# EBI-Metagenomics/deciphon

Measured on AMD Instinct MI355X. Metric: GCUPS (Viterbi DP cell updates/sec), higher is better.
Workload: dtype f32

## Files before the change

deciphon_amd/csrc/engine.cpp:

```cpp
#include "../../include/deciphon_hip.h"
#include "dcp_db.h"
#include "dcp_errors.h"
#include "dcp_types.h"
#include "host_logic.h"
#include "viterbi_kernels.h"

#include <algorithm>
#include <atomic>
#include <deque>
#include <math.h>
#include <stdio.h>
#include <stdlib.h>
#include <string.h>
#include <string>
#include <thread>
#include <vector>

namespace
{

template <class T> struct DevBuf
{
  T *p = nullptr;
  size_t cap = 0;
// ... 121 lines not shown
  size_t trellis_off = 0;
  bool has_trellis = false;
  bool trellis_on_host = false;
  uint32_t const *steps = nullptr;
  int32_t nsteps = 0;
  std::vector<uint32_t> owned;
};

}

struct dcp_hip
{
  int device = 0;
  hipStream_t stream = nullptr;
  hipStream_t qstream[DCP_NUM_CLASSES] = {nullptr};
  hipEvent_t fork_ev = nullptr, join_ev[DCP_NUM_CLASSES] = {nullptr};
  hipStream_t pstream[DCP_NUM_PACK_SHAPES] = {nullptr};
  hipEvent_t pjoin_ev[DCP_NUM_PACK_SHAPES] = {nullptr};
  hipStream_t nstream[DCP_NUM_CLASSES] = {nullptr};
  hipEvent_t njoin_ev[DCP_NUM_CLASSES] = {nullptr};
  std::string err;

  std::vector<HostProfile> profiles;
  size_t committed = 0;
  DevBuf<float> d_pool;
  size_t pool_used = 0;
  int load_chunks = 0;
  DevBuf<DcpProfileDev> d_profiles;

  std::vector<int64_t> seq_off, row_off;
  DevBuf<unsigned char> d_nt;
  DevBuf<int64_t> d_seq_off, d_row_off;
  DevBuf<DcpCodeRow> d_rows;

  bool mode_set = false;
  bool multi_hits = true, hmmer3_compat = false;
  DevBuf<float> d_xt;
  int xt_rows = 0;
  std::vector<float> xt_override;

  struct Bank
  {
    DevBuf<DcpProblem> d_problems;
    DevBuf<DcpPack> d_packs;
    DevBuf<int2> d_pack_groups;
    DevBuf<float> d_out;
    DevBuf<uint32_t> d_hits;
    DevBuf<float> d_ring;
    PinBuf<uint32_t> h_hits;
    hipEvent_t done_ev = nullptr;
    int n = -1;
    PinBuf<DcpProblem> h_problems;
    PinBuf<DcpPack> h_packs;
    PinBuf<int2> h_groups;
    hipEvent_t up_ev = nullptr;
    bool up_pending = false;
  };
  Bank bank[3];
  int cur = 0;
  int outstanding[2] = {-1, -1};
  hipStream_t upload_stream = nullptr;
  struct StreamSet
  {
    hipStream_t stream = nullptr, qstream[DCP_NUM_CLASSES] = {nullptr};
    hipEvent_t fork_ev = nullptr, join_ev[DCP_NUM_CLASSES] = {nullptr};
  } path_set;
// ... 318 lines not shown
  {
    HIP_TRY(x, B.h_problems.reserve((size_t)nu), DCP_ENOMEM);
    memcpy(B.h_problems.p, st.problems.data(), (size_t)nu * sizeof(DcpProblem));
    HIP_TRY(x, hipMemcpyAsync(B.d_problems.p, B.h_problems.p, (size_t)nu * sizeof(DcpProblem), hipMemcpyHostToDevice, origin),
            DCP_EFUNCUSE);
  }
  if (!st.packs.empty())
  {
    HIP_TRY(x, B.h_packs.reserve(st.packs.size()), DCP_ENOMEM);
    memcpy(B.h_packs.p, st.packs.data(), st.packs.size() * sizeof(DcpPack));
    HIP_TRY(x, hipMemcpyAsync(B.d_packs.p, B.h_packs.p, st.packs.size() * sizeof(DcpPack), hipMemcpyHostToDevice, origin),
            DCP_EFUNCUSE);
  }
  if (!st.pack_groups.empty())
  {
    HIP_TRY(x, B.h_groups.reserve(st.pack_groups.size()), DCP_ENOMEM);
    memcpy(B.h_groups.p, st.pack_groups.data(), st.pack_groups.size() * sizeof(int2));
    HIP_TRY(x, hipMemcpyAsync(B.d_pack_groups.p, B.h_groups.p, st.pack_groups.size() * sizeof(int2), hipMemcpyHostToDevice,
                              origin),
            DCP_EFUNCUSE);
  }
  HIP_TRY(x, hipEventRecord(B.up_ev, origin), DCP_EFUNCUSE);
  B.up_pending = true;
  return 0;
}

DcpLaunch launch_args(dcp_hip *x, Staged const &st, int c)
{
  DcpLaunch a;
  a.pool = x->d_pool.p;
  a.profiles = x->d_profiles.p;
  a.problems = BK(x).d_problems.p + st.c_begin[c];
  a.code_rows = x->d_rows.p;
  a.xt_table = x->d_xt.p;
  a.out = BK(x).d_out.p;
  a.arena = x->d_trellis.p;
  a.nprob = st.c_begin[c + 1] - st.c_begin[c];
  a.stream = x->stream;
  a.ring = BK(x).d_ring.p;
  return a;
}

int launch_all(dcp_hip *x, Staged const &st, bool path)
{
  int classes = 0;
  for (int c = 0; c < DCP_NUM_CLASSES; ++c) classes += st.c_begin[c + 1] > st.c_begin[c];
  bool const fork = classes > 1;
  if (fork) HIP_TRY(x, hipEventRecord(x->fork_ev, x->stream), DCP_EFUNCUSE);
  std::vector<hipEvent_t> joins;
  for (int c = 0; c < DCP_NUM_CLASSES; ++c)
  {
    DcpLaunch a = launch_args(x, st, c);
    if (a.nprob <= 0) continue;
    if (path && c == DCP_STRIP_CLASS) continue;
    if (fork)
    {
      a.stream = x->qstream[c];
      HIP_TRY(x, hipStreamWaitEvent(a.stream, x->fork_ev, 0), DCP_EFUNCUSE);
    }
    HIP_TRY(x, path ? dcp_launch_path(c, a) : dcp_launch_cost(c, a), DCP_EFUNCUSE);
    if (fork)
    {
      HIP_TRY(x, hipEventRecord(x->join_ev[c], a.stream), DCP_EFUNCUSE);
      joins.push_back(x->join_ev[c]);
    }
  }
  for (hipEvent_t ev : joins) HIP_TRY(x, hipStreamWaitEvent(x->stream, ev, 0), DCP_EFUNCUSE);
  return 0;
}

int launch_cost_all(dcp_hip *x, Staged const &st, hipStream_t origin = nullptr, int reps = 1)
{
  if (!origin) origin = x->stream;
  int const single_wave = st.c_begin[4] - st.c_begin[0];
  int mixed = 0;
  for (int c = 0; c < 4; ++c) mixed += st.c_begin[c + 1] > st.c_begin[c];
  bool const fused = mixed >= 2 && single_wave <= 16384;
  int kernels = fused ? 1 : 0;
  for (int c = fused ? 4 : 0; c < DCP_NUM_CLASSES; ++c) kernels += st.c_begin[c + 1] > st.c_begin[c];
  for (int s = 0; s < DCP_NUM_PACK_SHAPES; ++s) kernels += st.pk_begin[s + 1] > st.pk_begin[s];
  char const *narrow_env = getenv("DECIPHON_HIP_NARROW");
  bool const narrow = !(narrow_env && narrow_env[0] == '0');
  for (int c = 4; narrow && c < DCP_NUM_CLASSES; ++c) kernels += st.c_wide[c] > st.c_begin[c];
  bool const fork = kernels > 1 || origin != x->stream;
  if (fork) HIP_TRY(x, hipEventRecord(x->fork_ev, origin), DCP_EFUNCUSE);
  std::vector<hipEvent_t> joins;
  for (int c = DCP_NUM_CLASSES - 1; c >= (fused ? 4 : 0); --c)
  {
    DcpLaunch b = launch_args(x, st, c);
    if (b.nprob <= 0) continue;
    if (fork)
    {
      b.stream = x->qstream[c];
      HIP_TRY(x, hipStreamWaitEvent(b.stream, x->fork_ev, 0), DCP_EFUNCUSE);
    }
    int const nn = narrow ? st.c_wide[c] - st.c_begin[c] : 0;
    if (nn > 0)
    {
      DcpLaunch n = b;
      n.nprob = nn;
      if (fork)
      {
        n.stream = x->nstream[c];
        HIP_TRY(x, hipStreamWaitEvent(n.stream, x->fork_ev, 0), DCP_EFUNCUSE);
      }
      for (int r = 0; r < reps; ++r) HIP_TRY(x, dcp_launch_cost_narrow(c, n), DCP_EFUNCUSE);
      if (fork)
      {
        HIP_TRY(x, hipEventRecord(x->njoin_ev[c], n.stream), DCP_EFUNCUSE);
        joins.push_back(x->njoin_ev[c]);
      }
      b.problems += nn;
      b.nprob -= nn;
    }
    if (b.nprob > 0)
      for (int r = 0; r < reps; ++r) HIP_TRY(x, dcp_launch_cost(c, b), DCP_EFUNCUSE);
    if (fork)
// ... 450 lines not shown
    dev[i].W = hp.W;
    dev[i].rows_off = hp.pool_off;
    dev[i].trans_off = dev[i].rows_off + (int64_t)DCP_TABLE_SIZE * (hp.Kp + DCP_ROW_HDR);
    dev[i].pad0 = dev[i].pad1 = 0;
  }
  HIP_TRY(x, x->d_profiles.reserve(dev.size()), DCP_ENOMEM);
  HIP_TRY(x, hipMemcpyAsync(x->d_profiles.p, dev.data(), dev.size() * sizeof(DcpProfileDev), hipMemcpyHostToDevice,
                            x->stream),
          DCP_EFUNCUSE);
  HIP_TRY(x, hipStreamSynchronize(x->stream), DCP_EFUNCUSE);
  x->committed = x->profiles.size();
  return 0;
}

void dcp_hip_clear_profiles(struct dcp_hip *x)
{
  if (!x) return;
  x->pool_used = 0;
  x->profiles.clear();
  x->committed = 0;
}

int dcp_hip_encode(char const *data, int64_t n, uint8_t *out)
{
  if (n < 0 || (n > 0 && (!data || !out))) return DCP_EFUNCUSE;
  return dcp_encode_sequence(data, n, out);
}

int dcp_hip_set_sequences(struct dcp_hip *x, int nseq, uint8_t const *nt, int64_t const *offsets)
{
  if (!x || nseq < 0 || !offsets || (nseq > 0 && !nt)) return DCP_EFUNCUSE;
  if (outstanding_batches(x)) return fail(x, DCP_EFUNCUSE, "cost batches are outstanding (dcp_hip_cost_hits_begin): end them first");
  HIP_TRY(x, hipSetDevice(x->device), DCP_EFUNCUSE);
  x->seq_off.assign(offsets, offsets + nseq + 1);
  x->row_off.resize((size_t)nseq + 1);
  int64_t max_len = 0, rows = 0;
  if (x->seq_off[0] != 0) return fail(x, DCP_EFUNCUSE, "offsets[0] must be 0");
  for (int i = 0; i < nseq; ++i)
  {
    int64_t len = x->seq_off[(size_t)i + 1] - x->seq_off[(size_t)i];
    if (len < 0) return fail(x, DCP_EFUNCUSE, "offsets must not decrease");
    max_len = std::max(max_len, len);
    x->row_off[(size_t)i] = rows;
    rows += len + 1;
  }
  x->row_off[(size_t)nseq] = rows;
  int64_t const total = x->seq_off[(size_t)nseq];
  for (int64_t i = 0; i < total; ++i)
    if (nt[i] > 3) return fail(x, DCP_ESEQABC, "nucleotide index above 3");
  HIP_TRY(x, hipStreamSynchronize(x->stream), DCP_EFUNCUSE);
  HIP_TRY(x, x->d_nt.reserve((size_t)std::max<int64_t>(total, 1)), DCP_ENOMEM);
  HIP_TRY(x, x->d_seq_off.reserve((size_t)nseq + 1), DCP_ENOMEM);
  HIP_TRY(x, x->d_row_off.reserve((size_t)nseq + 1), DCP_ENOMEM);
  HIP_TRY(x, x->d_rows.reserve((size_t)std::max<int64_t>(rows, 1)), DCP_ENOMEM);
  if (total)
    HIP_TRY(x, hipMemcpyAsync(x->d_nt.p, nt, (size_t)total, hipMemcpyHostToDevice, x->stream), DCP_EFUNCUSE);
  HIP_TRY(x, hipMemcpyAsync(x->d_seq_off.p, x->seq_off.data(), ((size_t)nseq + 1) * sizeof(int64_t),
                            hipMemcpyHostToDevice, x->stream),
          DCP_EFUNCUSE);
  HIP_TRY(x, hipMemcpyAsync(x->d_row_off.p, x->row_off.data(), ((size_t)nseq + 1) * sizeof(int64_t),
                            hipMemcpyHostToDevice, x->stream),
          DCP_EFUNCUSE);
  HIP_TRY(x, dcp_launch_encode(x->d_nt.p, x->d_seq_off.p, x->d_row_off.p, nseq, max_len, x->d_rows.p, x->stream),
          DCP_EFUNCUSE);
  HIP_TRY(x, hipStreamSynchronize(x->stream), DCP_EFUNCUSE);
  return 0;
// ... 757 lines not shown
```

deciphon_amd/csrc/lane_ops_gpu.h:

```cpp
#pragma once
#include <hip/hip_runtime.h>
#include <stdint.h>
#include <type_traits>

#include "dcp_types.h"

#define DCP_FN __device__ __forceinline__
#define DCP_WAVE 64

typedef float lf;
typedef uint32_t lu;
typedef bool lm;

DCP_FN lf lf_splat(float x) { return x; }
DCP_FN lu lu_splat(uint32_t x) { return x; }
DCP_FN lf lmin(lf a, lf b) { return __builtin_fminf(a, b); }
DCP_FN lf lmin3(lf a, lf b, lf c) { return __builtin_fminf(__builtin_fminf(a, b), c); }
DCP_FN lm llt(lf a, lf b) { return a < b; }
DCP_FN lm llt_u(lu a, lu b) { return a < b; }
DCP_FN lm leq(lf a, lf b) { return a == b; }
DCP_FN lm lequ(lu a, lu b) { return a == b; }
DCP_FN lm land(lm a, lm b) { return a && b; }
DCP_FN lm lor(lm a, lm b) { return a || b; }
DCP_FN lm lnot(lm a) { return !a; }
// ... 3 lines not shown
DCP_FN lu lmaxu(lu a, lu b) { return a > b ? a : b; }

DCP_FN lu lane_ids() { return __builtin_amdgcn_mbcnt_hi(~0u, __builtin_amdgcn_mbcnt_lo(~0u, 0u)); }

DCP_FN lf lane_shift_up(lf x, float fill)
{
  return __int_as_float(
      __builtin_amdgcn_update_dpp(__float_as_int(fill), __float_as_int(x), 0x138, 0xf, 0xf, false));
}

DCP_FN lf lane_shift_up_keep(lf x, lf &keep)
{
  keep = __int_as_float(
      __builtin_amdgcn_update_dpp(__float_as_int(keep), __float_as_int(x), 0x138, 0xf, 0xf, false));
  return keep;
}

DCP_FN void sched_fence() { __builtin_amdgcn_sched_barrier(0); }
DCP_FN lf lf_pin(float x)
{
  lf v = x;
  asm volatile("" : "+v"(v));
  return v;
}

#define DCP_DPP_MIN_ALL(v, ctrl) \
  __builtin_fminf((v), __int_as_float(__builtin_amdgcn_update_dpp(0, __float_as_int(v), (ctrl), 0xf, 0xf, true)))
DCP_FN float wave_min(lf v)
{
  v = DCP_DPP_MIN_ALL(v, 0xB1);
  v = DCP_DPP_MIN_ALL(v, 0x4E);
  v = DCP_DPP_MIN_ALL(v, 0x141);
  v = DCP_DPP_MIN_ALL(v, 0x140);
  asm volatile("s_nop 1\n\tv_min_f32_dpp %0, %0, %0 row_bcast:15 row_mask:0xa bank_mask:0xf\n\t"
               "s_nop 1\n\tv_min_f32_dpp %0, %0, %0 row_bcast:31 row_mask:0xc bank_mask:0xf\n\t"
               "s_nop 1"
               : "+v"(v));
  return __int_as_float(__builtin_amdgcn_readlane(__float_as_int(v), 63));
}

DCP_FN uint32_t wave_minu(lu v)
{
  asm volatile("s_nop 1\n\tv_min_u32_dpp %0, %0, %0 row_shr:1 row_mask:0xf bank_mask:0xf\n\t"
               "s_nop 1\n\tv_min_u32_dpp %0, %0, %0 row_shr:2 row_mask:0xf bank_mask:0xf\n\t"
               "s_nop 1\n\tv_min_u32_dpp %0, %0, %0 row_shr:4 row_mask:0xf bank_mask:0xf\n\t"
               "s_nop 1\n\tv_min_u32_dpp %0, %0, %0 row_shr:8 row_mask:0xf bank_mask:0xf\n\t"
               "s_nop 1\n\tv_min_u32_dpp %0, %0, %0 row_bcast:15 row_mask:0xa bank_mask:0xf\n\t"
               "s_nop 1\n\tv_min_u32_dpp %0, %0, %0 row_bcast:31 row_mask:0xc bank_mask:0xf\n\t"
               "s_nop 1"
               : "+v"(v));
  return (uint32_t)__builtin_amdgcn_readlane((int)v, 63);
}

template <int P> DCP_FN void wave_priority() { __builtin_amdgcn_s_setprio(P); }

DCP_FN bool wave_any(lm m) { return __builtin_amdgcn_ballot_w64(m) != 0ull; }
DCP_FN uint64_t wave_ballot(lm m) { return __builtin_amdgcn_ballot_w64(m); }
DCP_FN float read_lane(lf x, int lane)
{
  return __int_as_float(__builtin_amdgcn_readlane(__float_as_int(x), lane));
}
DCP_FN uint32_t read_laneu(lu x, int lane) { return (uint32_t)__builtin_amdgcn_readlane((int)x, lane); }

enum { GS_M, GS_I, GS_D, GS_E, GS_F, GS_X, GS_T0, GS_T1, GS_X0, GS_X1, GS_SLOTS };

template <int Q> struct DcpStashChunk
{
  static constexpr int N = Q % 4 == 0 ? 4 : Q % 2 == 0 ? 2 : 1;
  typedef typename std::conditional<N == 4, float4, typename std::conditional<N == 2, float2, float>::type>::type type;
};
// ... 321 lines not shown
  float const *p = row + (size_t)lane * 5;
#pragma unroll
  for (int q = 0; q < 5; ++q) out[q] = p[q];
}
template <> DCP_FN void load_q<7>(float const *__restrict__ row, lu lane, lf (&out)[7])
{
  float const *p = row + (size_t)lane * 7;
#pragma unroll
  for (int q = 0; q < 7; ++q) out[q] = p[q];
}
template <> DCP_FN void load_q<6>(float const *__restrict__ row, lu lane, lf (&out)[6])
{
  float2 const *p = reinterpret_cast<float2 const *>(row + (size_t)lane * 6);
  float2 const a = p[0], b = p[1], c = p[2];
  out[0] = a.x; out[1] = a.y; out[2] = b.x; out[3] = b.y; out[4] = c.x; out[5] = c.y;
}
template <> DCP_FN void load_q<8>(float const *__restrict__ row, lu lane, lf (&out)[8])
{
  float4 const *p = reinterpret_cast<float4 const *>(row + (size_t)lane * 8);
  float4 const a = p[0], b = p[1];
  out[0] = a.x; out[1] = a.y; out[2] = a.z; out[3] = a.w; out[4] = b.x; out[5] = b.y; out[6] = b.z; out[7] = b.w;
}

template <> DCP_FN void load_q<10>(float const *__restrict__ row, lu lane, lf (&out)[10])
{
  float2 const *p = reinterpret_cast<float2 const *>(row + (size_t)lane * 10);
#pragma unroll
  for (int j = 0; j < 5; ++j)
  {
    float2 const a = p[j];
    out[2 * j] = a.x; out[2 * j + 1] = a.y;
  }
}
typedef unsigned int dcp_u32x2 __attribute__((ext_vector_type(2)));
typedef unsigned int dcp_u32x3 __attribute__((ext_vector_type(3)));
typedef unsigned int dcp_u32x4 __attribute__((ext_vector_type(4)));

struct RowSrc
{
  __amdgpu_buffer_rsrc_t rsrc;
  char const *base;
};

DCP_FN RowSrc rowsrc_make(float const *__restrict__ base, uint32_t bytes)
{
  RowSrc r;
  r.base = reinterpret_cast<char const *>(base);
  r.rsrc = __builtin_amdgcn_make_buffer_rsrc(const_cast<float *>(base), 0, (int)bytes, 0x00020000);
  return r;
}

template <int Q> DCP_FN lu row_lane_offset(lu lane) { return lane * (uint32_t)(Q * 4) + (uint32_t)(DCP_ROW_HDR * 4); }

DCP_FN void load_row_hdr(RowSrc const &r, uint32_t soff, float &nil, float &bg)
{
  float2 const h = *reinterpret_cast<float2 const *>(r.base + soff);
  nil = h.x;
  bg = h.y;
}

template <int Q> DCP_FN void load_row_q(RowSrc const &r, lu voff, uint32_t soff, lf (&out)[Q]);
template <> DCP_FN void load_row_q<1>(RowSrc const &r, lu voff, uint32_t soff, lf (&out)[1])
{
  out[0] = __uint_as_float(__builtin_amdgcn_raw_buffer_load_b32(r.rsrc, voff, soff, 0));
}
template <> DCP_FN void load_row_q<2>(RowSrc const &r, lu voff, uint32_t soff, lf (&out)[2])
// ... 315 lines not shown
```

deciphon_amd/csrc/viterbi_body.h:

```cpp
#pragma once
#include "dcp_types.h"

#ifndef DCP_FN
#error "include a lane_ops_*.h before viterbi_body.h"
#endif

#define DCP_INF (__builtin_inff())

#define DCP_SL(P, t) (((P) + 5 - (t)) % 5)

#ifndef DCP_LAZY_POSITIONS
#define DCP_LAZY_POSITIONS 6
#endif
constexpr int dcp_lazy_turns(int Q) { return Q >= DCP_LAZY_POSITIONS ? 1 : (DCP_LAZY_POSITIONS + Q - 1) / Q; }

#ifndef DCP_SHAPE_POLICY
#define DCP_SHAPE_POLICY(Q, W) ((W) == 1 ? ((Q) > 8 ? 7 : (Q) == 8 ? 2 : 0) : ((Q) >= 8 ? 6 : 0))
#endif
#ifndef DCP_COST_POLICY
#define DCP_COST_POLICY(Q, W) (DCP_SHAPE_POLICY(Q, W) | ((W) == 1 && ((Q) == 4 || (Q) == 5) ? 1 : 0))
#endif
template <int Q, int W, bool STORE = false, int POLICY = DCP_SHAPE_POLICY(Q, W)> struct CostWave
{
  static constexpr int TURNS = dcp_lazy_turns(Q);
  static constexpr bool LATE_FETCH = (POLICY & 1) != 0;
  static constexpr bool STASH = (POLICY & 6) != 0;
  static constexpr bool STASH6 = (POLICY & 4) != 0;
  static constexpr bool CHUNKED = STASH6 && W == 1;
  static constexpr int SLOTS = STASH6 ? 8 : 4;
  Group<W> g;
  float *__restrict__ tab_cells = nullptr;
  float *__restrict__ tab_sp = nullptr;
  int tabKp = 0;
  float *__restrict__ ckpt_out = nullptr;
  float const *__restrict__ ckpt_in = nullptr;
  int ckpt_every = 0;
  int row_base = 0;

  DCP_FN void save_ring(float *__restrict__ to)
  {
#pragma unroll
    for (int s = 0; s < 5; ++s)
    {
      store_q<Q>(to + (size_t)s * tabKp, g.lane, Mpre[s]);
      store_q<Q>(to + (size_t)(5 + s) * tabKp, g.lane, Ipre[s]);
      store_lane(to + (size_t)10 * tabKp + s * 64 * W, g.lane, Spre[s]);
    }
    store_lane(to + (size_t)10 * tabKp + 5 * 64 * W, g.lane, X);
  }
  DCP_FN void load_ring(float const *__restrict__ from)
  {
#pragma unroll
    for (int s = 0; s < 5; ++s)
    {
      load_q<Q>(from + (size_t)s * tabKp, g.lane, Mpre[s]);
      load_q<Q>(from + (size_t)(5 + s) * tabKp, g.lane, Ipre[s]);
      Spre[s] = load_lane(from + (size_t)10 * tabKp + s * 64 * W, g.lane);
    }
    X = load_lane(from + (size_t)10 * tabKp + 5 * 64 * W, g.lane);
  }
  lf BM[Q], MM[Q], MI[Q], MD[Q], IM[Q], II[Q], DM[Q], DD[Q];
  lf Mpre[5][Q], Ipre[5][Q], Spre[5];
  lf em[5][Q];
  lf sa, sb;
  lf X;
  lf NBv, EBv, JBv;
  lf shM, shI, shD;
  float nil[5], bgv[5];
  float ET, CT, RR;
  float E;
  RowSrc rows;
  lu voff;
  uint32_t stride_bytes;
  DcpCodeRow const *__restrict__ codes;

  DcpCodeRow cr;

  DCP_FN void fetch(int l_after, int L)
  {
#pragma unroll
    for (int t = 0; t < 5; ++t)
    {
      uint32_t const off = cr.c[t] * stride_bytes;
      load_row_hdr(rows, off, nil[t], bgv[t]);
      load_row_q<Q>(rows, voff, off, em[t]);
    }
    cr = codes[l_after <= L ? l_after : L];
  }

  DCP_FN void init(float const *__restrict__ pool, DcpProfileDev const &pf, DcpCodeRow const *__restrict__ code_rows,
                   float const *__restrict__ xt)
  {
#ifndef DCP_WAVE_PRIO
#define DCP_WAVE_PRIO(Q, W) ((W) > 1 || (Q) >= 6 ? 3 : (Q) >= 4 ? 2 : (Q) == 3 ? 1 : 0)
#endif
    wave_priority<DCP_WAVE_PRIO(Q, W)>();
    g.init();
    lu const lane = g.lane;
    int const Kp = pf.Kp;
    stride_bytes = (uint32_t)(Kp + DCP_ROW_HDR) * 4u;
    rows = rowsrc_make(pool + pf.rows_off, (uint32_t)DCP_TABLE_SIZE * stride_bytes);
    voff = row_lane_offset<Q>(lane);
    codes = code_rows;
    float const *__restrict__ trans = pool + pf.trans_off;
    load_q<Q>(trans + DCP_BM * Kp, lane, BM);
    load_q<Q>(trans + DCP_MM * Kp, lane, MM);
    load_q<Q>(trans + DCP_MI * Kp, lane, MI);
    load_q<Q>(trans + DCP_MD * Kp, lane, MD);
    load_q<Q>(trans + DCP_IM * Kp, lane, IM);
    load_q<Q>(trans + DCP_II * Kp, lane, II);
    load_q<Q>(trans + DCP_DM * Kp, lane, DM);
    load_q<Q>(trans + DCP_DD * Kp, lane, DD);
    NBv = lf_pin(xt[DCP_NB]);
    EBv = lf_pin(xt[DCP_EB]);
    JBv = lf_pin(xt[DCP_JB]);
    shM = shI = shD = lf_splat(DCP_INF);
    g.put_tdd(DD);
    if constexpr (STASH)
    {
      g.template stash_q<Q, SLOTS>(0, MD);
// ... 28 lines not shown
        Mpre[s][q] = inf;
        Ipre[s][q] = inf;
      }
    }
#pragma unroll
    for (int q = 0; q < Q; ++q) Mpre[0][q] = lf_splat(SB) + BM[q];
    Spre[0] = lsel(l0, lf_splat(0.0f + SN), lsel(l3, lf_splat(-RR + RR), inf));
    X = lsel(l3, lf_splat(-RR), inf);
    E = DCP_INF;
    tabKp = Kp;
    if (ckpt_in)
      load_ring(ckpt_in);
    else if (STORE)
      store_row0(SB);
  }

  template <int P> DCP_FN void row(int l, int L)
  {
    lf M[Q], I[Q];
#pragma unroll
    for (int q = 0; q < Q; ++q)
    {
      M[q] = lmin3(lmin3(Mpre[DCP_SL(P, 5)][q] + em[4][q], Mpre[DCP_SL(P, 4)][q] + em[3][q],
                         Mpre[DCP_SL(P, 3)][q] + em[2][q]),
                   Mpre[DCP_SL(P, 2)][q] + em[1][q], Mpre[DCP_SL(P, 1)][q] + em[0][q]);
      I[q] = lmin3(lmin3(Ipre[DCP_SL(P, 5)][q] + bgv[4], Ipre[DCP_SL(P, 4)][q] + bgv[3],
                         Ipre[DCP_SL(P, 3)][q] + bgv[2]),
                   Ipre[DCP_SL(P, 2)][q] + bgv[1], Ipre[DCP_SL(P, 1)][q] + bgv[0]);
    }
    X = lmin3(lmin3(Spre[DCP_SL(P, 5)] + nil[4], Spre[DCP_SL(P, 4)] + nil[3], Spre[DCP_SL(P, 3)] + nil[2]),
              Spre[DCP_SL(P, 2)] + nil[1], Spre[DCP_SL(P, 1)] + nil[0]);

    if constexpr (!LATE_FETCH)
      if (l < L) fetch(l + 2, L);

    lf m = M[0];
#pragma unroll
    for (int q = 1; q < Q; ++q) m = lmin(m, M[q]);
    lf D[Q];
    lf Msh0, Ish0, Dsh0, B;
    float N, J;
    if constexpr (STASH)
    {
      g.template unstash_q<Q, SLOTS>(0, MD);
      g.template unstash_q<Q, SLOTS>(1, DD);
    }
    if constexpr (W == 1)
    {
      Msh0 = lane_shift_up_keep(M[Q - 1], shM);
      Ish0 = lane_shift_up_keep(I[Q - 1], shI);
      E = wave_min(m);
      N = read_lane(X, 0);
      J = read_lane(X, 1);
      B = lmin3(N + NBv, E + EBv, J + JBv);

      D[0] = Msh0 + MD[0];
#pragma unroll
      for (int q = 1; q < Q; ++q) D[q] = lmin(M[q - 1] + MD[q], D[q - 1] + DD[q]);
      Dsh0 = lane_shift_up_keep(D[Q - 1], shD);
      lf x = Dsh0 + DD[0];
#pragma unroll
      for (int turn = 0; turn < TURNS; ++turn)
      {
        D[0] = lmin(D[0], x);
#pragma unroll
        for (int q = 1; q < Q; ++q) D[q] = lmin(D[q], D[q - 1] + DD[q]);
        Dsh0 = lane_shift_up_keep(D[Q - 1], shD);
// ... 60 lines not shown
      }
      else
      {
        g.note_fallback();
        D[0] = Msh0 + MD[0];
#pragma unroll
        for (int q = 1; q < Q; ++q) D[q] = lmin(M[q - 1] + MD[q], D[q - 1] + DD[q]);
        g.put_last(GS_D, D[Q - 1]);
        g.sync();
        Dsh0 = g.get_shift(GS_D, D[Q - 1], DCP_INF);
        x = Dsh0 + DD[0];
        better = llt(x, D[0]);
        g.put_any(GS_F, better);
        g.sync();
        while (g.get_any(GS_F, better))
        {
          D[0] = lmin(D[0], x);
#pragma unroll
          for (int q = 1; q < Q; ++q) D[q] = lmin(D[q], D[q - 1] + DD[q]);
          g.put_last(GS_D, D[Q - 1]);
          g.sync();
          Dsh0 = g.get_shift(GS_D, D[Q - 1], DCP_INF);
          x = Dsh0 + DD[0];
          better = llt(x, D[0]);
          g.put_any(GS_F, better);
          g.sync();
        }
      }
    }

    if constexpr (LATE_FETCH)
    {
      sched_fence();
      if (l < L) fetch(l + 2, L);
      sched_fence();
    }
    if constexpr (CHUNKED)
    {
      constexpr int N = DcpStashChunk<Q>::N;
#pragma unroll
      for (int j = 0; j < Q / N; ++j)
      {
        lf bm[N], mm[N], im[N], dm[N], ii[N], mi[N];
        g.template unstash_chunk<Q, SLOTS>(2, j, ii);
        g.template unstash_chunk<Q, SLOTS>(3, j, mi);
        g.template unstash_chunk<Q, SLOTS>(4, j, im);
        g.template unstash_chunk<Q, SLOTS>(5, j, dm);
        g.template unstash_chunk<Q, SLOTS>(6, j, bm);
        g.template unstash_chunk<Q, SLOTS>(7, j, mm);
#pragma unroll
        for (int i = 0; i < N; ++i)
        {
          int const q = N * j + i;
          lf const Ml = q ? M[q ? q - 1 : 0] : Msh0;
          lf const Il = q ? I[q ? q - 1 : 0] : Ish0;
          lf const Dl = q ? D[q ? q - 1 : 0] : Dsh0;
          Mpre[P][q] = lmin3(B + bm[i], Ml + mm[i], lmin(Il + im[i], Dl + dm[i]));
          Ipre[P][q] = lmin(I[q] + ii[i], M[q] + mi[i]);
        }
        sched_fence();
      }
    }
    else if constexpr (STASH)
    {
      g.template unstash_q<Q, SLOTS>(2, II);
      g.template unstash_q<Q, SLOTS>(3, MI);
      if constexpr (STASH6)
// ... 17 lines not shown
      }
    }
    Spre[P] = lmin(lf_splat(E) + sa, X + sb);
    if (STORE)
    {
      float *row = tab_cells + (size_t)(l - row_base) * 3 * (size_t)tabKp;
      store_q<Q>(row, g.lane, M);
      store_q<Q>(row + tabKp, g.lane, I);
      store_q<Q>(row + 2 * tabKp, g.lane, D);
      float const C = g.get_lane(GS_X0 + (l & 1), X, 2);
      store_sp_lane0(tab_sp + (size_t)(l - row_base) * DCP_SP_STRIDE, g.lane, lf_splat(N), B, lf_splat(J), lf_splat(E),
                     lf_splat(C));
    }
  }

  DCP_FN void store_row0(float SB)
  {
    lf inf[Q];
#pragma unroll
    for (int q = 0; q < Q; ++q) inf[q] = lf_splat(DCP_INF);
    store_q<Q>(tab_cells, g.lane, inf);
    store_q<Q>(tab_cells + tabKp, g.lane, inf);
    store_q<Q>(tab_cells + 2 * tabKp, g.lane, inf);
    lf const i = lf_splat(DCP_INF);
    store_sp_lane0(tab_sp, g.lane, i, lf_splat(SB), i, i, i);
  }

  DCP_FN void run(int L, float *out, int Lend = -1)
  {
    if (Lend < 0 || Lend > L) Lend = L;
    int l = row_base + 1;
    if (l <= Lend)
    {
      cr = codes[l];
      fetch(l + 1, Lend);
    }
    for (; l + 4 <= Lend; l += 5)
    {
      row<1>(l, Lend);
      row<2>(l + 1, Lend);
      row<3>(l + 2, Lend);
      row<4>(l + 3, Lend);
      row<0>(l + 4, Lend);
      if (ckpt_every > 0 && (l + 4) % ckpt_every == 0 && l + 4 + 5 < L)
        save_ring(ckpt_out + (size_t)((l + 4) / ckpt_every - 1) * (size_t)dcp_ckpt_floats(tabKp, W));
    }
    if (l <= Lend) row<1>(l++, Lend);
    if (l <= Lend) row<2>(l++, Lend);
    if (l <= Lend) row<3>(l++, Lend);
    if (l <= Lend) row<4>(l++, Lend);
    if (Lend < L) return;
    g.sync();
    g.put_lanes4(GS_X, X);
    g.sync();
    float const C = g.get_lane(GS_X, X, 2);
    float const R = g.get_lane(GS_X, X, 3);
    float const T = L > 0 ? __builtin_fminf(E + ET, C + CT) : DCP_INF;
    store_f32_lane0(out + 0, g.lane, R);
    store_f32_lane0(out + 1, g.lane, T);
  }
};

template <int Q, int W, bool STORE = false> struct StripWave
{
  Group<W> g;
  float *__restrict__ tab_cells = nullptr;
  float *__restrict__ tab_sp = nullptr;
// ... 458 lines not shown

    lf m = lmin(Ma[0], Da[0]);
#pragma unroll
    for (int q = 1; q < Q; ++q) m = lmin(m, lmin(Ma[q], Da[q]));
    g.put_min(GS_E, m);
    g.sync();
    Ea = g.get_min(GS_E, m);
    if (T == 1) pE = e_field(Ea, Ma, Da, Mbefore, Dbefore);

#pragma unroll
    for (int q = 1; q < Q; ++q) DCP_UPD(Da[q], pD[q], Da[q - 1] + DD[q], 1u);
    for (;;)
    {
      g.put_last(GS_D, Da[Q - 1]);
      g.sync();
      lf const x = g.get_shift(GS_D, Da[Q - 1], DCP_INF) + DD[0];
      lm const better = llt(x, Da[0]);
      g.put_any(GS_F, better);
      g.sync();
      if (!g.get_any(GS_F, better)) break;
      DCP_UPD(Da[0], pD[0], x, 1u);
#pragma unroll
      for (int q = 1; q < Q; ++q) DCP_UPD(Da[q], pD[q], Da[q - 1] + DD[q], 1u);
    }

    DCP_UPDS(Ba, pB, Ea + xt[DCP_EB], 2u);
    DCP_UPDS(Ba, pB, Ja + xt[DCP_JB], 3u);
    DCP_UPDS(Ta, pT, Ea + xt[DCP_ET], 0u);
    DCP_UPDS(Ta, pT, Ca + xt[DCP_CT], 1u);
  }

  DCP_FN void fetch(int l_after, int L)
  {
#pragma unroll
    for (int t = 0; t < 5; ++t)
    {
      uint32_t const off = cr.c[t] * stride_bytes;
      load_row_hdr(rows, off, nil[t], bgv[t]);
      load_row_q<Q>(rows, voff, off, em[t]);
    }
    cr = codes[l_after <= L ? l_after : L];
  }

  template <int P> DCP_FN float row(int l, int L)
  {
    lf const inf = lf_splat(DCP_INF);
    lf Ma[Q], Ia[Q], Da[Q];
    lu pM[Q], pI[Q], pD[Q];
#pragma unroll
    for (int q = 0; q < Q; ++q)
    {
      Ma[q] = Ia[q] = Da[q] = inf;
      pM[q] = pI[q] = pD[q] = lu_splat(0);
    }
    float Na = DCP_INF, Ba = DCP_INF, Ja = DCP_INF, Ea = DCP_INF, Ca = DCP_INF, Ta = DCP_INF;
    uint32_t pN = 0, pB = 0, pJ = 0, pE = 0, pC = 0, pT = 0;

    if (l >= 5) pass<5, DCP_SL(P, 5)>(l, Ma, Ia, Da, pM, pI, pD, Na, Ba, Ja, Ea, Ca, Ta, pN, pB, pJ, pE, pC, pT);
    if (l >= 4) pass<4, DCP_SL(P, 4)>(l, Ma, Ia, Da, pM, pI, pD, Na, Ba, Ja, Ea, Ca, Ta, pN, pB, pJ, pE, pC, pT);
    if (l >= 3) pass<3, DCP_SL(P, 3)>(l, Ma, Ia, Da, pM, pI, pD, Na, Ba, Ja, Ea, Ca, Ta, pN, pB, pJ, pE, pC, pT);
    if (l >= 2) pass<2, DCP_SL(P, 2)>(l, Ma, Ia, Da, pM, pI, pD, Na, Ba, Ja, Ea, Ca, Ta, pN, pB, pJ, pE, pC, pT);
    pass<1, DCP_SL(P, 1)>(l, Ma, Ia, Da, pM, pI, pD, Na, Ba, Ja, Ea, Ca, Ta, pN, pB, pJ, pE, pC, pT);
    if (l < L) fetch(l + 2, L);

    lu const lane = g.lane;
    store_u32_lane0(xnodes + l, lane, (pN << 0) | (pB << 4) | (pE << 6) | (pC << 21) | (pT << 25) | (pJ << 26));
    lu w[Q];
#pragma unroll
    for (int q = 0; q < Q; ++q)
    {
      lu const k = lane * (uint32_t)Q + (uint32_t)q;
      lu word = pM[q];
      word = word | lselu(lequ(k, lu_splat(0)), lu_splat(0), pD[q] << 5);
      word = word | lselu(llt_u(k + 1u, lu_splat((uint32_t)K)), pI[q] << 6, lu_splat(0));
      w[q] = word;
    }
    store_nodes_q<Q>(nodes + (size_t)l * (size_t)K, K, lane, w);

#pragma unroll
    for (int q = 0; q < Q; ++q)
    {
      M[P][q] = Ma[q];
      I[P][q] = Ia[q];
      D[P][q] = Da[q];
    }
    g.put_last(GS_M, Ma[Q - 1]);
    g.put_last(GS_I, Ia[Q - 1]);
    g.put_last(GS_D, Da[Q - 1]);
    g.sync();
    Msh[P] = g.get_shift(GS_M, Ma[Q - 1], DCP_INF);
    Ish[P] = g.get_shift(GS_I, Ia[Q - 1], DCP_INF);
    Dsh[P] = g.get_shift(GS_D, Da[Q - 1], DCP_INF);
    S[P] = DCP_INF;
    N[P] = Na;
    B[P] = Ba;
    J[P] = Ja;
    E[P] = Ea;
    C[P] = Ca;
    return Ta;
  }

  DCP_FN float run(int L)
  {
    float T = DCP_INF;
    if (L > 0)
    {
      cr = codes[1];
      fetch(2, L);
    }
    int l = 1;
    for (; l + 4 <= L; l += 5)
    {
      T = row<1>(l, L);
      T = row<2>(l + 1, L);
      T = row<3>(l + 2, L);
      T = row<4>(l + 3, L);
      T = row<0>(l + 4, L);
    }
    if (l <= L) T = row<1>(l++, L);
    if (l <= L) T = row<2>(l++, L);
    if (l <= L) T = row<3>(l++, L);
    if (l <= L) T = row<4>(l++, L);
    return T;
  }
};
```

deciphon_amd/csrc/viterbi_kernels.h:

```cpp
#pragma once
#include "dcp_types.h"
#include <hip/hip_runtime.h>

#define DCP_NUM_CLASSES 12
#define DCP_STRIP_CLASS 11
#define DCP_STRIP_POSITIONS 2048
#define DCP_MAX_CORE_SIZE 16383
#define DCP_RING_FLOATS ((size_t)10 * DCP_MAX_STRIPS * DCP_STRIP_POSITIONS)
#define DCP_RING_SLOTS 1024
int dcp_class_of(int K);
void dcp_class_shape(int cls, int *Q, int *W);

#define DCP_NUM_PACK_SHAPES 11
int dcp_pack_shape_of(int K);
void dcp_pack_shape(int shape, int *Q, int *S);

struct DcpLaunch
{
  float const *pool;
  DcpProfileDev const *profiles;
  DcpProblem const *problems;
  DcpCodeRow const *code_rows;
  float const *xt_table;
  float *out;
  unsigned char *arena;
  float *ring = nullptr;
  int nprob;
  hipStream_t stream;
};

hipError_t dcp_launch_cost(int cls, DcpLaunch const &a);
int dcp_class_narrow_limit(int cls);
hipError_t dcp_launch_cost_narrow(int cls, DcpLaunch const &a);
hipError_t dcp_launch_path(int cls, DcpLaunch const &a);
hipError_t dcp_launch_unzip(DcpLaunch const &a, uint32_t *steps, int64_t const *step_off, int32_t *nsteps);
hipError_t dcp_launch_cost_ckpt(int cls, DcpLaunch const &a, int64_t const *ckpt_addr, int B);
hipError_t dcp_launch_cost_store(int cls, DcpLaunch const &a, int64_t const *ckpt_addr, int B, int block, int G = 0, int it = 0);
hipError_t dcp_launch_traceback(DcpLaunch const &a, uint32_t *steps, int64_t const *step_off, int32_t *nsteps,
                                DcpTraceState *states, int B, int block, int G = 0, int it = 0);
hipError_t dcp_launch_path_blocks(int cls, DcpLaunch const &a, int64_t const *ckpt_addr, int B, uint32_t *steps,
                                  int64_t const *step_off, int32_t *nsteps, DcpTraceState *states);
hipError_t dcp_launch_replay(DcpLaunch const &a, int64_t const *table_addr, int64_t const *scratch_addr, int max_rows);
hipError_t dcp_launch_compact_steps(uint32_t const *steps, int64_t const *step_off, int64_t const *compact_off,
                                    uint32_t *out, int n, hipStream_t stream);
hipError_t dcp_launch_cost_pack(int shape, DcpLaunch const &a, DcpPack const *packs, int npack, uint32_t ncode_rows);
hipError_t dcp_launch_lrt_filter(float const *out, int n, uint32_t *hits, hipStream_t stream);
int dcp_pack_lds_waves(int shape);
hipError_t dcp_launch_cost_pack_lds(int shape, DcpLaunch const &a, DcpPack const *packs, int2 const *groups, int ngroups,
                                    uint32_t ncode_rows);
hipError_t dcp_launch_cost_fused(DcpLaunch const &a);
hipError_t dcp_launch_encode(unsigned char const *nt, int64_t const *seq_off, int64_t const *row_off, int nseq,
                             int64_t max_len, DcpCodeRow *rows, hipStream_t stream);
```

deciphon_amd/csrc/viterbi_kernels.hip:

```cpp
#include <stdlib.h>

#include "lane_ops_gpu.h"
#include "viterbi_body.h"
#include "viterbi_pack.h"
#include "traceback.h"
#include "viterbi_kernels.h"
#include "row_replay.h"

template <class T> __device__ __forceinline__ T *dcp_global(uintptr_t address)
{
  return (T *)(__attribute__((address_space(1))) T *)address;
}

__device__ __forceinline__ int dcp_xcd_remap_any(int b, int n)
{
  int const q = n >> 3, r = n & 7, x = b & 7;
  return (x < r ? x * (q + 1) : r * (q + 1) + (x - r) * q) + (b >> 3);
}
__device__ __forceinline__ int dcp_xcd_remap(int b, int n)
{
  return n < 16384 ? b : dcp_xcd_remap_any(b, n);
}

#ifndef DCP_COST_WAVES
#define DCP_COST_WAVES(Q, W) ((W) == 1 && (Q) == 4 ? 4 : (W) == 1 && (Q) == 5 ? 3 : (Q) >= 8 ? 2 : 1)
#endif
template <int Q, int W, int POLICY = DCP_COST_POLICY(Q, W), int WAVES = DCP_COST_WAVES(Q, W)>
__global__ __launch_bounds__(64 * W, WAVES) void dcp_cost_kernel(float const *__restrict__ pool,
                                                      DcpProfileDev const *__restrict__ profiles,
                                                      DcpProblem const *__restrict__ problems,
                                                      DcpCodeRow const *__restrict__ code_rows,
                                                      float const *__restrict__ xt_table,
                                                      float *__restrict__ out, int nprob)
{
  if ((int)blockIdx.x >= nprob) return;
#ifdef DCP_EXP_LDSPAD
  __shared__ float pad[DCP_EXP_LDSPAD / 4];
  if (nprob < 0) out[0] = pad[threadIdx.x];
#endif
  int const p = dcp_xcd_remap((int)blockIdx.x, nprob);
  DcpProblem const pb = problems[p];
  DcpProfileDev const pf = profiles[pb.profile];
  CostWave<Q, W, false, POLICY> w;
  w.init(pool, pf, code_rows + pb.code_row, xt_table + (size_t)pb.xt_row * DCP_XT_STRIDE);
  w.run(pb.L, out + 2 * (size_t)pb.out);
}

template <int Q, int W>
__global__ __launch_bounds__(64 * W, (Q >= 8 ? 2 : 1)) void dcp_cost_ckpt_kernel(float const *__restrict__ pool,
                                                           DcpProfileDev const *__restrict__ profiles,
                                                           DcpProblem const *__restrict__ problems,
                                                           DcpCodeRow const *__restrict__ code_rows,
                                                           float const *__restrict__ xt_table,
                                                           int64_t const *__restrict__ ckpt_addr, int B,
                                                           float *__restrict__ out, int nprob)
{
  if ((int)blockIdx.x >= nprob) return;
  DcpProblem const pb = problems[dcp_xcd_remap_any((int)blockIdx.x, nprob)];
  if (dcp_num_blocks(pb.L, B) <= 1) return;
  DcpProfileDev const pf = profiles[pb.profile];
  CostWave<Q, W> w;
  w.ckpt_out = dcp_global<float>((uintptr_t)ckpt_addr[pb.out]);
  w.ckpt_every = B;
  w.init(pool, pf, code_rows + pb.code_row, xt_table + (size_t)pb.xt_row * DCP_XT_STRIDE);
  w.run(pb.L, out + 2 * (size_t)pb.out);
}

template <int Q, int W>
__global__ __launch_bounds__(64 * W, (Q >= 8 ? 2 : 1)) void dcp_cost_store_kernel(float const *__restrict__ pool,
                                                            DcpProfileDev const *__restrict__ profiles,
                                                            DcpProblem const *__restrict__ problems,
                                                            DcpCodeRow const *__restrict__ code_rows,
                                                            float const *__restrict__ xt_table,
                                                            unsigned char *__restrict__ arena,
                                                            int64_t const *__restrict__ ckpt_addr, int B, int block,
                                                            int G, int it, float *__restrict__ out, int nprob)
{
// ... 487 lines not shown
  PathWave<Q, W> w;
  w.init(pool, pf, code_rows + pb.code_row, xt_table + (size_t)pb.xt_row * DCP_XT_STRIDE, xnodes, nodes);
  float const T = w.run(pb.L);
  store_f32_lane0(out + pb.out, w.g.lane, T);
}

__global__ void dcp_encode_kernel(unsigned char const *__restrict__ nt, int64_t const *__restrict__ seq_off,
                                  int64_t const *__restrict__ row_off, int nseq, DcpCodeRow *__restrict__ rows)
{
  for (int s = (int)blockIdx.y; s < nseq; s += (int)gridDim.y)
  {
    int64_t const n = seq_off[s + 1] - seq_off[s];
    unsigned char const *x = nt + seq_off[s];
    DcpCodeRow *out = rows + row_off[s];
    for (int64_t r = (int64_t)blockIdx.x * blockDim.x + threadIdx.x; r <= n; r += (int64_t)gridDim.x * blockDim.x)
    {
      DcpCodeRow cr;
      unsigned const off[5] = {0u, 4u, 20u, 84u, 340u};
      unsigned idx = 0;
#pragma unroll
      for (int t = 1; t <= 5; ++t)
      {
        bool const ok = r - t >= 0;
        unsigned const sym = ok ? x[r - t] : 0u;
        idx += sym << (2 * (t - 1));
        cr.c[t - 1] = ok ? off[t - 1] + idx : 0u;
      }
      cr.c[5] = cr.c[6] = cr.c[7] = 0;
      out[r] = cr;
    }
  }
}

__global__ void dcp_unzip_kernel(DcpProfileDev const *__restrict__ profiles, DcpProblem const *__restrict__ problems,
                                 unsigned char const *__restrict__ arena, uint32_t *__restrict__ steps,
                                 int64_t const *__restrict__ step_off, int32_t *__restrict__ nsteps, int nprob)
{
  int const p = (int)(blockIdx.x * blockDim.x + threadIdx.x);
  if (p >= nprob) return;
  DcpProblem const pb = problems[p];
  int const K = profiles[pb.profile].K;
  int const L = pb.L;
  uint32_t const *xnodes = reinterpret_cast<uint32_t const *>(arena + pb.trellis);
  uint16_t const *nodes = reinterpret_cast<uint16_t const *>(xnodes + (L + 1));
  uint32_t *buf = steps + step_off[pb.out];
  int64_t const cap = step_off[pb.out + 1] - step_off[pb.out];
  enum
  {
    ST_M = 0 << 14, ST_I = 1 << 14, ST_D = 2 << 14, ST_X = 3 << 14,
    ST_S = ST_X | 3, ST_N = ST_X | 4, ST_B = ST_X | 5, ST_E = ST_X | 6, ST_J = ST_X | 7, ST_C = ST_X | 8, ST_T = ST_X | 9,
  };
  int state = ST_T, stage = L;
  int64_t n = 0;
  bool bad = false;
  while ((state != ST_S || stage) && !bad)
  {
    int size = 0, prev = 0;
    if ((state & ST_X) == ST_X)
    {
      uint32_t const x = xnodes[stage];
      if (state == ST_N) { unsigned v = x & 0xF; size = (int)(v % 5) + 1; prev = v / 5 ? ST_N : ST_S; }
      else if (state == ST_B) { unsigned v = (x >> 4) & 0x3; prev = v == 0 ? ST_S : v == 1 ? ST_N : v == 2 ? ST_E : ST_J; }
      else if (state == ST_E) { unsigned v = (x >> 6) & 0x7FFF; prev = (v & 1 ? ST_D : ST_M) | (int)(v / 2 + 1); }
      else if (state == ST_C) { unsigned v = (x >> 21) & 0xF; size = (int)(v % 5) + 1; prev = v / 5 ? ST_C : ST_E; }
      else if (state == ST_T) { unsigned v = (x >> 25) & 0x1; prev = v ? ST_C : ST_E; }
      else if (state == ST_J) { unsigned v = (x >> 26) & 0xF; size = (int)(v % 5) + 1; prev = v / 5 ? ST_J : ST_E; }
// ... 78 lines not shown

__global__ void dcp_compact_steps_kernel(uint32_t const *__restrict__ steps, int64_t const *__restrict__ step_off,
                                         int64_t const *__restrict__ compact_off, uint32_t *__restrict__ out, int n)
{
  int const i = (int)blockIdx.x;
  if (i >= n) return;
  int64_t const count = compact_off[i + 1] - compact_off[i];
  uint32_t const *src = steps + step_off[i + 1] - count;
  uint32_t *dst = out + compact_off[i];
  for (int64_t j = threadIdx.x; j < count; j += blockDim.x) dst[j] = src[j];
}

hipError_t dcp_launch_compact_steps(uint32_t const *steps, int64_t const *step_off, int64_t const *compact_off,
                                    uint32_t *out, int n, hipStream_t stream)
{
  if (n <= 0) return hipSuccess;
  hipLaunchKernelGGL(dcp_compact_steps_kernel, dim3((unsigned)n), dim3(256), 0, stream, steps, step_off, compact_off,
                     out, n);
  return hipGetLastError();
}

hipError_t dcp_launch_unzip(DcpLaunch const &a, uint32_t *steps, int64_t const *step_off, int32_t *nsteps)
{
  if (a.nprob <= 0) return hipSuccess;
  unsigned const blocks = (unsigned)((a.nprob + 63) / 64);
  hipLaunchKernelGGL(dcp_unzip_kernel, dim3(blocks), dim3(64), 0, a.stream, a.profiles, a.problems, a.arena, steps,
                     step_off, nsteps, a.nprob);
  return hipGetLastError();
}

template <int Q, int W, int POLICY = DCP_COST_POLICY(Q, W), int WAVES = DCP_COST_WAVES(Q, W)>
static hipError_t launch_cost_qw(DcpLaunch const &a)
{
  hipLaunchKernelGGL((dcp_cost_kernel<Q, W, POLICY, WAVES>), dim3((unsigned)a.nprob), dim3(64 * W), 0, a.stream, a.pool,
                     a.profiles, a.problems, a.code_rows, a.xt_table, a.out, a.nprob);
  return hipGetLastError();
}

template <int Q, int W> static hipError_t launch_path_qw(DcpLaunch const &a)
{
  hipLaunchKernelGGL((dcp_path_kernel<Q, W>), dim3((unsigned)a.nprob), dim3(64 * W), 0, a.stream, a.pool, a.profiles,
                     a.problems, a.code_rows, a.xt_table, a.arena, a.out, a.nprob);
  return hipGetLastError();
}

template <bool STORE> static hipError_t launch_strip(DcpLaunch const &a)
{
  if (!a.ring) return hipErrorInvalidValue;
  unsigned const grid = (unsigned)(a.nprob < DCP_RING_SLOTS ? a.nprob : DCP_RING_SLOTS);
  hipLaunchKernelGGL((dcp_strip_kernel<4, 8, STORE>), dim3(grid), dim3(512), 0, a.stream, a.pool,
                     a.profiles, a.problems, a.code_rows, a.xt_table, a.arena, a.ring, a.out, a.nprob);
  return hipGetLastError();
}

int dcp_class_of(int K)
{
  if (K < 1) return -1;
  if (K <= 256) return K > 60 && K <= 64 ? 1 : (K + 63) / 64 - 1;
  if (K <= 384) return 4;
  if (K <= 512) return 5;
  if (K <= 768) return 6;
  if (K <= 1024) return 7;
  if (K <= 1536) return 8;
  if (K <= 2048) return 9;
  if (K <= 4096) return 10;
  if (K <= DCP_MAX_CORE_SIZE) return DCP_STRIP_CLASS;
  return -1;
}
// ... 224 lines not shown
}

hipError_t dcp_launch_path(int cls, DcpLaunch const &a)
{
  if (a.nprob <= 0) return hipSuccess;
  switch (cls)
  {
  case 0: return launch_path_qw<1, 1>(a);
  case 1: return launch_path_qw<2, 1>(a);
  case 2: return launch_path_qw<3, 1>(a);
  case 3: return launch_path_qw<4, 1>(a);
  case 4: return launch_path_qw<3, 2>(a);
  case 5: return launch_path_qw<4, 2>(a);
  case 6: return launch_path_qw<3, 4>(a);
  case 7: return launch_path_qw<4, 4>(a);
  case 8: return launch_path_qw<3, 8>(a);
  case 9: return launch_path_qw<4, 8>(a);
  case 10: return launch_path_qw<4, 16>(a);
  default: return hipErrorInvalidValue;
  }
}

hipError_t dcp_launch_encode(unsigned char const *nt, int64_t const *seq_off, int64_t const *row_off, int nseq,
                             int64_t max_len, DcpCodeRow *rows, hipStream_t stream)
{
  if (nseq <= 0) return hipSuccess;
  unsigned bx = (unsigned)((max_len + 1 + 255) / 256);
  if (bx < 1) bx = 1;
  if (bx > 1024) bx = 1024;
  hipLaunchKernelGGL(dcp_encode_kernel, dim3(bx, (unsigned)(nseq < 65535 ? nseq : 65535)), dim3(256), 0, stream, nt,
                     seq_off, row_off, nseq, rows);
  return hipGetLastError();
}
```

Before: 813.7.

## Precompute per-class scaled code-row byte offsets and load code rows as vectors

Adds a per-class device table of code-row indices pre-multiplied by the emission row stride, built once per sequence set by a new scale kernel. The cost kernel reads these scaled offsets directly, which removes a multiply per fetch and the clamp branch on the next row index; two spare rows are padded on so reads past the end stay in bounds. Code rows are loaded as a single 8-dword vector and pinned to scalar registers. The wave-min reduction's inline-asm row_bcast steps are replaced with DPP builtins. In exchange the change costs extra device memory per class, a one-time preprocessing launch, and the cost kernel launch now fails with an error if no offset table was prepared.

```diff
diff --git a/deciphon_amd/csrc/engine.cpp b/deciphon_amd/csrc/engine.cpp
--- a/deciphon_amd/csrc/engine.cpp
+++ b/deciphon_amd/csrc/engine.cpp
@@ -177,6 +177,8 @@
   DevBuf<unsigned char> d_nt;
   DevBuf<int64_t> d_seq_off, d_row_off;
   DevBuf<DcpCodeRow> d_rows;
+  DevBuf<DcpCodeRow> d_offs[DCP_NUM_CLASSES];
+  bool offs_ok[DCP_NUM_CLASSES] = {false};
 
   bool mode_set = false;
   bool multi_hits = true, hmmer3_compat = false;
@@ -561,6 +563,7 @@
   a.profiles = x->d_profiles.p;
   a.problems = BK(x).d_problems.p + st.c_begin[c];
   a.code_rows = x->d_rows.p;
+  a.row_offs = x->offs_ok[c] ? x->d_offs[c].p : nullptr;
   a.xt_table = x->d_xt.p;
   a.out = BK(x).d_out.p;
   a.arena = x->d_trellis.p;
@@ -595,6 +598,19 @@
     }
   }
   for (hipEvent_t ev : joins) HIP_TRY(x, hipStreamWaitEvent(x->stream, ev, 0), DCP_EFUNCUSE);
+  return 0;
+}
+
+int ensure_row_offs(dcp_hip *x, int c, hipStream_t s)
+{
+  if (x->offs_ok[c]) return 0;
+  int Q, W;
+  dcp_class_shape(c, &Q, &W);
+  int64_t const rows = x->row_off.back();
+  HIP_TRY(x, x->d_offs[c].reserve((size_t)rows + DCP_SPARE_ROWS), DCP_ENOMEM);
+  HIP_TRY(x, dcp_launch_scale_rows(x->d_rows.p, rows, (uint32_t)(64 * Q * W + DCP_ROW_HDR) * 4u, x->d_offs[c].p, s),
+          DCP_EFUNCUSE);
+  x->offs_ok[c] = true;
   return 0;
 }
 
@@ -612,6 +628,9 @@
   bool const narrow = !(narrow_env && narrow_env[0] == '0');
   for (int c = 4; narrow && c < DCP_NUM_CLASSES; ++c) kernels += st.c_wide[c] > st.c_begin[c];
   bool const fork = kernels > 1 || origin != x->stream;
+  for (int c = fused ? 4 : 0; c < DCP_STRIP_CLASS; ++c)
+    if (st.c_begin[c + 1] > st.c_begin[c])
+      if (int rc = ensure_row_offs(x, c, origin)) return rc;
   if (fork) HIP_TRY(x, hipEventRecord(x->fork_ev, origin), DCP_EFUNCUSE);
   std::vector<hipEvent_t> joins;
   for (int c = DCP_NUM_CLASSES - 1; c >= (fused ? 4 : 0); --c)
@@ -1128,6 +1147,7 @@
   if (!x || nseq < 0 || !offsets || (nseq > 0 && !nt)) return DCP_EFUNCUSE;
   if (outstanding_batches(x)) return fail(x, DCP_EFUNCUSE, "cost batches are outstanding (dcp_hip_cost_hits_begin): end them first");
   HIP_TRY(x, hipSetDevice(x->device), DCP_EFUNCUSE);
+  for (bool &ok : x->offs_ok) ok = false;
   x->seq_off.assign(offsets, offsets + nseq + 1);
   x->row_off.resize((size_t)nseq + 1);
   int64_t max_len = 0, rows = 0;
diff --git a/deciphon_amd/csrc/lane_ops_gpu.h b/deciphon_amd/csrc/lane_ops_gpu.h
--- a/deciphon_amd/csrc/lane_ops_gpu.h
+++ b/deciphon_amd/csrc/lane_ops_gpu.h
@@ -59,10 +59,8 @@
   v = DCP_DPP_MIN_ALL(v, 0x4E);
   v = DCP_DPP_MIN_ALL(v, 0x141);
   v = DCP_DPP_MIN_ALL(v, 0x140);
-  asm volatile("s_nop 1\n\tv_min_f32_dpp %0, %0, %0 row_bcast:15 row_mask:0xa bank_mask:0xf\n\t"
-               "s_nop 1\n\tv_min_f32_dpp %0, %0, %0 row_bcast:31 row_mask:0xc bank_mask:0xf\n\t"
-               "s_nop 1"
-               : "+v"(v));
+  v = DCP_DPP_MIN_ALL(v, 0x142);
+  v = DCP_DPP_MIN_ALL(v, 0x143);
   return __int_as_float(__builtin_amdgcn_readlane(__float_as_int(v), 63));
 }
 
@@ -450,6 +448,24 @@
     out[2 * j] = a.x; out[2 * j + 1] = a.y;
   }
 }
+#define DCP_HAVE_CODE_ROW_LOAD 1
+typedef unsigned int dcp_u32x8 __attribute__((ext_vector_type(8)));
+DCP_FN DcpCodeRow code_row_load(DcpCodeRow const *__restrict__ p)
+{
+  dcp_u32x8 const v = *reinterpret_cast<dcp_u32x8 const *>(p);
+  DcpCodeRow r;
+  r.c[0] = v.s0; r.c[1] = v.s1; r.c[2] = v.s2; r.c[3] = v.s3;
+  r.c[4] = v.s4; r.c[5] = v.s5; r.c[6] = v.s6; r.c[7] = v.s7;
+  return r;
+}
+DCP_FN void code_row_ready(DcpCodeRow &r)
+{
+  dcp_u32x8 v = {r.c[0], r.c[1], r.c[2], r.c[3], r.c[4], r.c[5], r.c[6], r.c[7]};
+  asm("" : "+s"(v));
+  r.c[0] = v.s0; r.c[1] = v.s1; r.c[2] = v.s2; r.c[3] = v.s3;
+  r.c[4] = v.s4; r.c[5] = v.s5; r.c[6] = v.s6; r.c[7] = v.s7;
+}
+
 typedef unsigned int dcp_u32x2 __attribute__((ext_vector_type(2)));
 typedef unsigned int dcp_u32x3 __attribute__((ext_vector_type(3)));
 typedef unsigned int dcp_u32x4 __attribute__((ext_vector_type(4)));
diff --git a/deciphon_amd/csrc/viterbi_body.h b/deciphon_amd/csrc/viterbi_body.h
--- a/deciphon_amd/csrc/viterbi_body.h
+++ b/deciphon_amd/csrc/viterbi_body.h
@@ -20,7 +20,13 @@
 #ifndef DCP_COST_POLICY
 #define DCP_COST_POLICY(Q, W) (DCP_SHAPE_POLICY(Q, W) | ((W) == 1 && ((Q) == 4 || (Q) == 5) ? 1 : 0))
 #endif
-template <int Q, int W, bool STORE = false, int POLICY = DCP_SHAPE_POLICY(Q, W)> struct CostWave
+
+#ifndef DCP_HAVE_CODE_ROW_LOAD
+DCP_FN DcpCodeRow code_row_load(DcpCodeRow const *__restrict__ p) { return *p; }
+DCP_FN void code_row_ready(DcpCodeRow &) {}
+#endif
+
+template <int Q, int W, bool STORE = false, int POLICY = DCP_SHAPE_POLICY(Q, W), bool SCALED = false> struct CostWave
 {
   static constexpr int TURNS = dcp_lazy_turns(Q);
   static constexpr bool LATE_FETCH = (POLICY & 1) != 0;
@@ -78,14 +84,15 @@
 
   DCP_FN void fetch(int l_after, int L)
   {
+    code_row_ready(cr);
 #pragma unroll
     for (int t = 0; t < 5; ++t)
     {
-      uint32_t const off = cr.c[t] * stride_bytes;
+      uint32_t const off = SCALED ? cr.c[t] : cr.c[t] * stride_bytes;
       load_row_hdr(rows, off, nil[t], bgv[t]);
       load_row_q<Q>(rows, voff, off, em[t]);
     }
-    cr = codes[l_after <= L ? l_after : L];
+    cr = code_row_load(codes + (SCALED ? l_after : l_after <= L ? l_after : L));
   }
 
   DCP_FN void init(float const *__restrict__ pool, DcpProfileDev const &pf, DcpCodeRow const *__restrict__ code_rows,
@@ -180,7 +187,7 @@
               Spre[DCP_SL(P, 2)] + nil[1], Spre[DCP_SL(P, 1)] + nil[0]);
 
     if constexpr (!LATE_FETCH)
-      if (l < L) fetch(l + 2, L);
+      if (SCALED || l < L) fetch(l + 2, L);
 
     lf m = M[0];
 #pragma unroll
@@ -307,7 +314,7 @@
     if constexpr (LATE_FETCH)
     {
       sched_fence();
-      if (l < L) fetch(l + 2, L);
+      if (SCALED || l < L) fetch(l + 2, L);
       sched_fence();
     }
     if constexpr (CHUNKED)
@@ -391,7 +398,7 @@
     int l = row_base + 1;
     if (l <= Lend)
     {
-      cr = codes[l];
+      cr = code_row_load(codes + l);
       fetch(l + 1, Lend);
     }
     for (; l + 4 <= Lend; l += 5)
@@ -916,6 +923,7 @@
 
   DCP_FN void fetch(int l_after, int L)
   {
+    code_row_ready(cr);
 #pragma unroll
     for (int t = 0; t < 5; ++t)
     {
@@ -923,7 +931,7 @@
       load_row_hdr(rows, off, nil[t], bgv[t]);
       load_row_q<Q>(rows, voff, off, em[t]);
     }
-    cr = codes[l_after <= L ? l_after : L];
+    cr = code_row_load(codes + (l_after <= L ? l_after : L));
   }
 
   template <int P> DCP_FN float row(int l, int L)
@@ -989,7 +997,7 @@
     float T = DCP_INF;
     if (L > 0)
     {
-      cr = codes[1];
+      cr = code_row_load(codes + 1);
       fetch(2, L);
     }
     int l = 1;
diff --git a/deciphon_amd/csrc/viterbi_kernels.h b/deciphon_amd/csrc/viterbi_kernels.h
--- a/deciphon_amd/csrc/viterbi_kernels.h
+++ b/deciphon_amd/csrc/viterbi_kernels.h
@@ -21,6 +21,7 @@
   DcpProfileDev const *profiles;
   DcpProblem const *problems;
   DcpCodeRow const *code_rows;
+  DcpCodeRow const *row_offs = nullptr;
   float const *xt_table;
   float *out;
   unsigned char *arena;
@@ -49,5 +50,8 @@
 hipError_t dcp_launch_cost_pack_lds(int shape, DcpLaunch const &a, DcpPack const *packs, int2 const *groups, int ngroups,
                                     uint32_t ncode_rows);
 hipError_t dcp_launch_cost_fused(DcpLaunch const &a);
+#define DCP_SPARE_ROWS 2
+hipError_t dcp_launch_scale_rows(DcpCodeRow const *rows, int64_t nrows, uint32_t stride_bytes, DcpCodeRow *out,
+                                 hipStream_t stream);
 hipError_t dcp_launch_encode(unsigned char const *nt, int64_t const *seq_off, int64_t const *row_off, int nseq,
                              int64_t max_len, DcpCodeRow *rows, hipStream_t stream);
diff --git a/deciphon_amd/csrc/viterbi_kernels.hip b/deciphon_amd/csrc/viterbi_kernels.hip
--- a/deciphon_amd/csrc/viterbi_kernels.hip
+++ b/deciphon_amd/csrc/viterbi_kernels.hip
@@ -29,7 +29,7 @@
 __global__ __launch_bounds__(64 * W, WAVES) void dcp_cost_kernel(float const *__restrict__ pool,
                                                       DcpProfileDev const *__restrict__ profiles,
                                                       DcpProblem const *__restrict__ problems,
-                                                      DcpCodeRow const *__restrict__ code_rows,
+                                                      DcpCodeRow const *__restrict__ row_offs,
                                                       float const *__restrict__ xt_table,
                                                       float *__restrict__ out, int nprob)
 {
@@ -41,8 +41,8 @@
   int const p = dcp_xcd_remap((int)blockIdx.x, nprob);
   DcpProblem const pb = problems[p];
   DcpProfileDev const pf = profiles[pb.profile];
-  CostWave<Q, W, false, POLICY> w;
-  w.init(pool, pf, code_rows + pb.code_row, xt_table + (size_t)pb.xt_row * DCP_XT_STRIDE);
+  CostWave<Q, W, false, POLICY, true> w;
+  w.init(pool, pf, row_offs + pb.code_row, xt_table + (size_t)pb.xt_row * DCP_XT_STRIDE);
   w.run(pb.L, out + 2 * (size_t)pb.out);
 }
 
@@ -596,6 +596,23 @@
   }
 }
 
+__global__ void dcp_scale_rows_kernel(DcpCodeRow const *__restrict__ rows, int64_t nrows, uint32_t stride_bytes,
+                                      DcpCodeRow *__restrict__ out)
+{
+  for (int64_t r = (int64_t)blockIdx.x * blockDim.x + threadIdx.x; r < nrows + DCP_SPARE_ROWS;
+       r += (int64_t)gridDim.x * blockDim.x)
+  {
+    DcpCodeRow o = {};
+    if (r < nrows)
+    {
+      DcpCodeRow const cr = rows[r];
+#pragma unroll
+      for (int t = 0; t < 5; ++t) o.c[t] = cr.c[t] * stride_bytes;
+    }
+    out[r] = o;
+  }
+}
+
 __global__ void dcp_unzip_kernel(DcpProfileDev const *__restrict__ profiles, DcpProblem const *__restrict__ problems,
                                  unsigned char const *__restrict__ arena, uint32_t *__restrict__ steps,
                                  int64_t const *__restrict__ step_off, int32_t *__restrict__ nsteps, int nprob)
@@ -740,8 +757,9 @@
 template <int Q, int W, int POLICY = DCP_COST_POLICY(Q, W), int WAVES = DCP_COST_WAVES(Q, W)>
 static hipError_t launch_cost_qw(DcpLaunch const &a)
 {
+  if (!a.row_offs) return hipErrorInvalidValue;
   hipLaunchKernelGGL((dcp_cost_kernel<Q, W, POLICY, WAVES>), dim3((unsigned)a.nprob), dim3(64 * W), 0, a.stream, a.pool,
-                     a.profiles, a.problems, a.code_rows, a.xt_table, a.out, a.nprob);
+                     a.profiles, a.problems, a.row_offs, a.xt_table, a.out, a.nprob);
   return hipGetLastError();
 }
 
@@ -1032,3 +1050,12 @@
                      seq_off, row_off, nseq, rows);
   return hipGetLastError();
 }
+
+hipError_t dcp_launch_scale_rows(DcpCodeRow const *rows, int64_t nrows, uint32_t stride_bytes, DcpCodeRow *out,
+                                 hipStream_t stream)
+{
+  int64_t const blocks = (nrows + DCP_SPARE_ROWS + 255) / 256;
+  hipLaunchKernelGGL(dcp_scale_rows_kernel, dim3((unsigned)(blocks < 4096 ? blocks : 4096)), dim3(256), 0, stream, rows,
+                     nrows, stride_bytes, out);
+  return hipGetLastError();
+}
```

Result: faster. 828.6, median of 6 (+1.8%).
